# vt-asaplab/porla

Measured on NVIDIA B200. Metric: G1 MSM points/sec, higher is better.
Workload: dtype u32 (8x32-bit limb Montgomery, IMAD carry chains)

## Files before the change

porla_b200/csrc/msm_impl.cuh:

```cuda
#pragma once
#include <atomic>
#include <cstdio>
#include <cstdlib>
#include <mutex>
#include <type_traits>

#include "arena.h"
#include "msm.h"
#include "msm_kernels.cuh"
#include "small_kernels.cuh"
#include "affine_kernels.cuh"

namespace porla {

extern std::atomic<uint64_t> g_launches;
#define LAUNCHED() (g_launches.fetch_add(1, std::memory_order_relaxed))



template <class C> struct CurveIdOf;
template <> struct CurveIdOf<Bn254> { static constexpr int value = kCurveBn254; };
template <> struct CurveIdOf<Secp256k1> { static constexpr int value = kCurveSecp256k1; };

template <class C>
void import_into_impl(const uint8_t* d_bytes, int fmt, uint32_t n, void* d_points_out, uint8_t* d_flags_out,
                      cudaStream_t stream, bool with_phi) {
    using F = typename C::F;
    if (!n) return;
    int mask = C::F::Params::kMontgomery ? 1 : 0;
    k_import_points<C><<<(n + 127) / 128, 128, 0, stream>>>(d_bytes, fmt, mask, n, reinterpret_cast<Affine<F>*>(d_points_out),
                                                           d_flags_out, nullptr);
    LAUNCHED();
    if constexpr (C::kGlv) {
        if (with_phi) {
            k_phi_table<C><<<(n + 127) / 128, 128, 0, stream>>>(reinterpret_cast<const Affine<F>*>(d_points_out), n,
                                                               reinterpret_cast<F*>(reinterpret_cast<Affine<F>*>(d_points_out) + n));
            LAUNCHED();
        }
    }
    PORLA_CUDA(cudaGetLastError());
}

template <class C>
void import_impl(const uint8_t* d_bytes, int fmt, uint32_t n, PointTable* out, cudaStream_t stream) {
    using F = typename C::F;
    Affine<F>* pts = nullptr;
    uint8_t* flags = nullptr;
    uint32_t* d_count = nullptr;
    PORLA_CUDA(cudaMalloc(&pts, (size_t)(n ? n : 1) * (sizeof(Affine<F>) + (C::kGlv ? sizeof(F) : 0))));
    PORLA_CUDA(cudaMalloc(&flags, (size_t)(n ? n : 1)));
    PORLA_CUDA(cudaMalloc(&d_count, 4));
    PORLA_CUDA(cudaMemsetAsync(d_count, 0, 4, stream));
    if (n) {
        int mask = C::F::Params::kMontgomery ? 1 : 0;
        k_import_points<C><<<(n + 127) / 128, 128, 0, stream>>>(d_bytes, fmt, mask, n, pts, flags, d_count);
        LAUNCHED();
        if constexpr (C::kGlv) {
            k_phi_table<C><<<(n + 127) / 128, 128, 0, stream>>>(pts, n, reinterpret_cast<F*>(pts + n));
            LAUNCHED();
        }
        PORLA_CUDA(cudaGetLastError());
    }
    uint32_t h_count = 0;
    PORLA_CUDA(cudaMemcpyAsync(&h_count, d_count, 4, cudaMemcpyDeviceToHost, stream));
    PORLA_CUDA(cudaStreamSynchronize(stream));
    PORLA_CUDA(cudaFree(d_count));
    out->d_points = pts;
    out->n = n;
    out->n_inf = h_count;
    out->curve = CurveIdOf<C>::value;
    out->phi_off = C::kGlv ? n : 0u;
    out->d_phi_x = C::kGlv ? static_cast<void*>(pts + n) : nullptr;
    if (h_count == 0) {
        PORLA_CUDA(cudaFree(flags));
        out->d_flags = nullptr;
    } else {
        out->d_flags = flags;
    }
}

template <class C>
void msm_small_impl(const PointTable& table, const uint8_t* d_scalars, uint32_t n, uint32_t nbatch, const MsmOptions& opt,
                    const MsmPlan& plan, uint8_t* d_out, void* d_out_xyzz, cudaStream_t stream) {
    using F = typename C::F;
    using XC = XYZZ<typename C::FC>;
    const bool lut = plan.mode == kPlanLut;
    const uint32_t slots = nbatch * (uint32_t)plan.nwin;
    uint32_t K = 1, nblk;
    if (lut) {
        uint32_t per_thread = 1;
        if (nbatch > 8) {
            const uint64_t want_threads = 148ull * 3 * kTreeThreads * 4;
            per_thread = (uint32_t)(((uint64_t)n * nbatch) / want_threads);
            if (per_thread < 1) per_thread = 1;
            if (per_thread > 16) per_thread = 16;
            while (per_thread > 1 && n / per_thread < (uint32_t)kTreeThreads) per_thread >>= 1;
        }
        K = nbatch > 8 ? (uint32_t)table.fb_nwin * per_thread : 2u;
        const uint32_t threads = (n * (uint32_t)table.fb_nwin + K - 1) / K;
        nblk = (threads + kTreeThreads - 1) / kTreeThreads;
    } else {
        nblk = (n + 2 * kTreeThreads - 1) / (2 * kTreeThreads);
    }
    if (!nblk) nblk = 1;
    const size_t need = Arena::padded((size_t)slots * nblk, sizeof(XYZZ<F>)) + Arena::padded(slots, 4) +
                        Arena::padded(slots, sizeof(XYZZ<F>)) + 1024;
    DeviceCtx& cx = device_ctx();
    Arena& g_arena = cx.arena;
    StageTimer& g_stage_timer = cx.timer;
    std::unique_lock<std::mutex> lock(cx.engine_mu, std::defer_lock);
    XYZZ<F>* partials;
    uint32_t* tickets;
    XYZZ<F>* wsum;
    if (opt.d_scratch && need <= opt.scratch_bytes) {
        uint8_t* b = reinterpret_cast<uint8_t*>(opt.d_scratch);
        partials = reinterpret_cast<XYZZ<F>*>(b);
        b += Arena::padded((size_t)slots * nblk, sizeof(XYZZ<F>));
        tickets = reinterpret_cast<uint32_t*>(b);
        b += Arena::padded(slots, 4);
        wsum = reinterpret_cast<XYZZ<F>*>(b);
    } else {
        lock.lock();
        g_arena.acquire(stream);
        g_arena.reserve(need, stream);
        g_arena.reset();
        partials = g_arena.take<XYZZ<F>>((size_t)slots * nblk);
        tickets = g_arena.take<uint32_t>(slots);
        wsum = g_arena.take<XYZZ<F>>(slots);
    }
    for (int st = kStageCount; st <= kStageAccumulate; st++) g_stage_timer.mark(st, stream);
    if (nblk > 1) PORLA_CUDA(cudaMemsetAsync(tickets, 0, (size_t)slots * 4, stream));
    if (lut) {
        const int m_major = nbatch > 8 ? 1 : 0;
        k_lut_sum<C><<<m_major ? dim3(nbatch, nblk) : dim3(nblk, nbatch), kTreeThreads, 0, stream>>>(
            reinterpret_cast<const Affine<F>*>(table.d_lut), table.fb_c, table.fb_nwin, d_scalars, opt.scalar_be, n, K, m_major,
            partials, tickets, wsum);
    } else {
        k_small_bits<C><<<dim3(nblk, (uint32_t)plan.nwin, nbatch), kTreeThreads, 0, stream>>>(
            reinterpret_cast<const Affine<F>*>(table.d_points), table.d_flags, d_scalars, opt.scalar_be, n, opt.shared_points,
            partials, tickets, wsum);
    }
    LAUNCHED();
    g_stage_timer.mark(kStageReduce, stream);
    g_stage_timer.mark(kStageFinalize, stream);
    if (opt.d_window_sums) {
        PORLA_CUDA(cudaMemcpyAsync(opt.d_window_sums, wsum, (size_t)slots * sizeof(XYZZ<F>), cudaMemcpyDeviceToDevice, stream));
    } else {
        k_finalize<C><<<(nbatch + 31) / 32, 32, 0, stream>>>((const XC*)wsum, nbatch, plan.nwin, plan.c, opt.out_fmt, d_out,
                                                            reinterpret_cast<XC*>(d_out_xyzz));
        LAUNCHED();
    }
    g_stage_timer.mark(kNumStages, stream);
    if (lock.owns_lock()) g_arena.release(stream);
    PORLA_CUDA(cudaGetLastError());
}

template <class C>
void msm_impl(const PointTable& table, const uint8_t* d_scalars, uint32_t n, uint32_t nbatch,
                     const MsmOptions& opt, uint8_t* d_out, void* d_out_xyzz, cudaStream_t stream) {
    using F = typename C::F;
    const int curve = CurveIdOf<C>::value;
    {
        const MsmPlan plan = msm_plan_table(table, n, nbatch, opt);
        if (plan.mode != kPlanPipeline && n > 0) {
            msm_small_impl<C>(table, d_scalars, n, nbatch, opt, plan, d_out, d_out_xyzz, stream);
            return;
        }
    }
    MsmShape sh;
    sh.n = n;
    sh.nbatch = nbatch;
    sh.shared = opt.shared_points ? 1u : 0u;
    const bool streamed = opt.part_mode != kPartWhole;
    if (streamed && (nbatch != 1 || !opt.d_buckets || opt.window_bits <= 0 || opt.glv < 0 || !opt.no_fixed_base)) {
        fprintf(stderr, "[libmultiexp/porla_b200] FATAL: a streamed MSM part needs one MSM, a shared bucket array and a forced window layout\n");
        abort();
    }
    const bool fixed = table.fb_c > 0 && opt.shared_points && !opt.no_fixed_base &&
                       (opt.window_bits == 0 || opt.window_bits == table.fb_c);
    const MsmPlan wplan = fixed ? MsmPlan{table.fb_c, 1, kPlanPipeline, 0} : msm_plan(curve, n, nbatch, opt.window_bits, opt.glv);
    const bool glv = wplan.glv != 0;
    if (glv && !(C::kGlv && table.phi_off && table.d_phi_x)) {
        fprintf(stderr, "[libmultiexp/porla_b200] FATAL: GLV plan for a table without its endomorphism image\n");
        abort();
    }
    sh.c = wplan.c;
    sh.nwin = glv ? 2 * wplan.nwin : (C::kScalarBits + 1 + sh.c - 1) / sh.c;
    int slice_shift = 0;
    while ((1 << slice_shift) < opt.slice_count) slice_shift++;
    if (opt.slice_count > 1) {
        const bool ok = (1 << slice_shift) == opt.slice_count && opt.slice_index >= 0 && opt.slice_index < opt.slice_count &&
                        !fixed && nbatch == 1 && opt.window_bits > 0 && opt.glv >= 0 && opt.no_fixed_base &&
                        msm_max_slices(wplan, opt.slice_count) == opt.slice_count;
        if (!ok) {
            fprintf(stderr, "[libmultiexp/porla_b200] FATAL: bucket slice %d of %d: needs one MSM, a forced window layout and a power-of-two "
                            "slice count that leaves whole coarse bins (c = %d)\n", opt.slice_index, opt.slice_count, wplan.c);
            abort();
        }
    }
    sh.slice_shift = (uint32_t)slice_shift;
    sh.slice_r = opt.slice_count > 1 ? (uint32_t)opt.slice_index : 0u;
    sh.nbuckets = (1u << (sh.c - 1)) >> slice_shift;
    sh.fixed_n = fixed ? table.fb_n : 0u;
    sh.glv_wh = glv ? wplan.nwin : 0;
    sh.phi_off = glv ? table.phi_off : 0u;
    const int slot_windows = fixed ? 1 : (glv ? wplan.nwin : sh.nwin);

    const uint64_t slots = (uint64_t)nbatch * slot_windows;
    const uint64_t nbt64 = slots * sh.nbuckets;
    const uint64_t pairs64 = (uint64_t)nbatch * n * sh.nwin;
    if (nbt64 >= (1ull << 32) || pairs64 >= (1ull << 32) || (uint64_t)nbatch * n >= (1ull << 31) ||
        (fixed && (uint64_t)table.fb_n * sh.nwin >= (1ull << 31))) {
        fprintf(stderr, "[libmultiexp/porla_b200] FATAL: MSM shape too large for 32-bit indexing\n");
        abort();
    }
    const uint32_t nbt = (uint32_t)nbt64;
    const uint32_t ntiles = (nbt + kScanTile - 1) / kScanTile;

    uint32_t chunk = 64;
    while (chunk > 4 && (uint64_t)nbt / chunk < 24576ull) chunk >>= 1;
    while (chunk > 4 && sh.nbuckets / chunk < 4) chunk >>= 1;
    if (const char* e = getenv("PORLA_REDUCE_CHUNK")) { if (atoi(e) >= 1) chunk = (uint32_t)atoi(e); }
    if (chunk > sh.nbuckets) chunk = sh.nbuckets;
    uint32_t threads_per_slot = (sh.nbuckets + chunk - 1) / chunk;
    uint32_t blocks_per_slot = (threads_per_slot + kRedThreads - 1) / kRedThreads;
    static const uint64_t quad_max = [] { const char* e = getenv("PORLA_REDUCE_QUAD_MAX"); return e ? (uint64_t)atoll(e) : (uint64_t)C::kReduceQuadMax; }();
    static const uint64_t quad_target = [] { const char* e = getenv("PORLA_REDUCE_QUADS"); return e && atoll(e) > 0 ? (uint64_t)atoll(e) : 148ull * kQuadsPerBlock; }();
    const bool reduce_v1 = getenv("PORLA_REDUCE_V1") != nullptr || (uint64_t)nbt > quad_max;
    uint32_t log_m = 0;
    while (log_m < 6 && ((uint64_t)nbt >> log_m) > quad_target) log_m++;
    while ((sh.nbuckets >> log_m) > (uint32_t)(kTopMaxBlocks * kQuadsPerBlock)) log_m++;
    while (log_m > 0 && (1u << log_m) > sh.nbuckets) log_m--;
    const uint32_t scan_tps = sh.nbuckets >> log_m;
    const uint32_t scan_group = scan_tps >= (uint32_t)kQuadsPerBlock ? (uint32_t)kQuadsPerBlock : scan_tps;
    const uint32_t scan_bps = scan_tps >= (uint32_t)kQuadsPerBlock ? scan_tps / kQuadsPerBlock : 1u;
    if (!reduce_v1) blocks_per_slot = 2 * scan_bps;

    const uint64_t pairs_cap = pairs64 ? pairs64 : 1;
    const uint64_t pairs_geo = (pairs_cap >> slice_shift) ? (pairs_cap >> slice_shift) : 1;
    const uint64_t wave = 148ull * 4ull * kAccThreads;
    const uint64_t waves = (pairs_geo + wave * 64 - 1) / (wave * 64);
    uint32_t L = (uint32_t)((pairs_geo + waves * wave - 1) / (waves * wave));
    if (waves == 1) {
        const uint64_t l2 = pairs_geo / (wave * 18 / 25);
        if (l2 >= 16 && l2 <= 64) L = (uint32_t)l2;
    }
    if (L < 16) L = 16;
    if (L > 64) L = 64;
    if (const char* e = getenv("PORLA_SLICE_LEN")) { if (atoi(e) >= 2) L = (uint32_t)atoi(e); }
    int aff_rounds = 0;
    {
        const char* e = getenv("PORLA_ACC_AFFINE");
        const bool big = pairs_cap >= (uint64_t)148 * PORLA_AFF_MIN_BLOCKS * kAffThreads * kAffL * 2;
        const int want = e ? atoi(e) : (big ? kAffDefaultRounds : 0);
        if (want > 0 && !streamed && slice_shift == 0) {
            aff_rounds = want > 2 ? 2 : want;
            L = kAffL;
        }
    }
    const uint32_t nslices_cap = (uint32_t)((pairs_cap + L - 1) / L);
    const uint32_t serial_limit = (nslices_cap >> slice_shift) < 200000u ? kStitchSerialSmall : kStitchSerial;
    const uint32_t long_cap = (uint32_t)(pairs_cap / ((uint64_t)L * serial_limit)) + 2;

    const bool radix = nbatch == 1 && n >= (1u << 19) && sh.nwin <= 28 && sh.c >= 9 && sh.c <= 20 && (sh.nbuckets >> (sh.c / 2)) <= (uint32_t)kPartMaxBins && !getenv("PORLA_ATOMIC_SCATTER");
    const int lb = sh.c / 2;
    const uint32_t ncoarse = radix ? (nbt >> lb) : 0u;
    DeviceCtx& cx = device_ctx();
    Arena& g_arena = cx.arena;
    StageTimer& g_stage_timer = cx.timer;
    std::lock_guard<std::mutex> lock(cx.engine_mu);
    size_t need = (radix ? Arena::padded(pairs_cap, 8) + Arena::padded(ncoarse, 4) : 0) + Arena::padded(nbt, 4) * 2 + Arena::padded(ntiles + 1, 4) + 512 +
                  Arena::padded(pairs_cap, 8) + (streamed ? 0 : Arena::padded(nbt, sizeof(XYZZ<F>))) +
                  2 * Arena::padded(nslices_cap, sizeof(XYZZ<F>)) + Arena::padded(long_cap, 8) +
                  Arena::padded(slots * blocks_per_slot, sizeof(XYZZ<F>)) + Arena::padded(slots, sizeof(XYZZ<F>));
    g_arena.acquire(stream);
    g_arena.reserve(need, stream);
    g_arena.reset();
    uint32_t* counters = g_arena.take<uint32_t>(nbt);
    uint32_t* offsets = g_arena.take<uint32_t>(nbt);
    uint32_t* tile_sums = g_arena.take<uint32_t>(ntiles + 1);
    uint32_t* grand = g_arena.take<uint32_t>(1);
    uint32_t* long_count = g_arena.take<uint32_t>(1);
    uint2* sorted = g_arena.take<uint2>(pairs_cap);
    uint2* part = radix ? g_arena.take<uint2>(pairs_cap) : nullptr;
    uint32_t* coarse_cursor = radix ? g_arena.take<uint32_t>(ncoarse) : nullptr;
    XYZZ<F>* buckets = streamed ? reinterpret_cast<XYZZ<F>*>(opt.d_buckets) : g_arena.take<XYZZ<F>>(nbt);
    const int into = opt.part_mode == kPartMiddle || opt.part_mode == kPartLast;
    XYZZ<F>* part_head = g_arena.take<XYZZ<F>>(nslices_cap);
    XYZZ<F>* part_tail = g_arena.take<XYZZ<F>>(nslices_cap);
    uint2* long_runs = g_arena.take<uint2>(long_cap);
    XYZZ<F>* partials = g_arena.take<XYZZ<F>>(slots * blocks_per_slot);
    XYZZ<F>* wsum = g_arena.take<XYZZ<F>>(slots);

    const Affine<F>* points = reinterpret_cast<const Affine<F>*>(fixed ? table.d_fb_points : table.d_points);
    using FC = typename C::FC;
    using XC = XYZZ<FC>;
    static_assert(sizeof(XC) == sizeof(XYZZ<F>), "layouts must coincide");
    const uint64_t total_scalars = (uint64_t)n * nbatch;

    g_stage_timer.mark(kStageCount, stream);
    const char* sv2 = getenv("PORLA_SORT_V2");
    const bool v2_fits = ncoarse > 0 && pairs_cap / ncoarse <= (uint64_t)(kBigBin * 0.95);
    const bool sort_v2 = radix && slice_shift == 0 && lb <= 10 && (size_t)ncoarse * 4 <= (160u << 10) && (sv2 ? sv2[0] == '1' : v2_fits);
    PORLA_CUDA(cudaMemsetAsync(counters, 0, (size_t)nbt * 4, stream));
    PORLA_CUDA(cudaMemsetAsync(grand, 0, 4, stream));
    PORLA_CUDA(cudaMemsetAsync(long_count, 0, 4, stream));
    static_assert(sizeof(XYZZ<F>) == 128, "k_fine_smem / k_big_scan clear 128-byte bucket records");
    if (!into && !sort_v2) PORLA_CUDA(cudaMemsetAsync(buckets, 0, (size_t)nbt * sizeof(XYZZ<F>), stream));
    uint4* zero_buckets = into ? nullptr : reinterpret_cast<uint4*>(buckets);
    if (total_scalars && sort_v2) {
        static std::once_flag attr_once_dev2[kMaxDevices];
        const size_t smem0 = (size_t)ncoarse * 4;
        const size_t smem1 = ((size_t)9 * kPartTile + 2 * kPartMaxBins) * 4 + (size_t)kPartTile * 8;
        const size_t smem2 = (size_t)2 * kFineHist * 4 + (size_t)kFineTile * 8;
        const size_t smem3 = (size_t)kBigBin * 6 + (size_t)kFineLocalBuckets * 4;
        std::call_once(attr_once_dev2[current_device()], [=] {
            PORLA_CUDA(cudaFuncSetAttribute(k_coarse_count<C, false>, cudaFuncAttributeMaxDynamicSharedMemorySize, 160 << 10));
            PORLA_CUDA(cudaFuncSetAttribute(k_partition_coarse<C, false>, cudaFuncAttributeMaxDynamicSharedMemorySize, (int)smem1));
            if constexpr (C::kGlv) {
                PORLA_CUDA(cudaFuncSetAttribute(k_coarse_count<C, true>, cudaFuncAttributeMaxDynamicSharedMemorySize, 160 << 10));
                PORLA_CUDA(cudaFuncSetAttribute(k_partition_coarse<C, true>, cudaFuncAttributeMaxDynamicSharedMemorySize, (int)smem1));
            }
            PORLA_CUDA(cudaFuncSetAttribute(k_partition_fine_big, cudaFuncAttributeMaxDynamicSharedMemorySize, (int)smem2));
            PORLA_CUDA(cudaFuncSetAttribute(k_fine_smem, cudaFuncAttributeMaxDynamicSharedMemorySize, (int)smem3));
        });
        uint32_t* coarse_count = offsets;
        uint32_t* coarse_off = offsets + ncoarse + 1;
        PORLA_CUDA(cudaMemsetAsync(coarse_count, 0, (size_t)(ncoarse + 1) * 4, stream));
        uint32_t cgrid = (uint32_t)((total_scalars + kCoarseCountThreads - 1) / kCoarseCountThreads);
        if (cgrid > 148u * 2u) cgrid = 148u * 2u;
        bool glv_done = false;
        if constexpr (C::kGlv) {
            if (glv) {
                k_coarse_count<C, true><<<cgrid, kCoarseCountThreads, smem0, stream>>>(d_scalars, opt.scalar_be, table.d_flags, sh, lb, ncoarse, coarse_count);
                glv_done = true;
            }
        }
        if (!glv_done)
            k_coarse_count<C, false><<<cgrid, kCoarseCountThreads, smem0, stream>>>(d_scalars, opt.scalar_be, table.d_flags, sh, lb, ncoarse, coarse_count);
        LAUNCHED();
        g_stage_timer.mark(kStageScan, stream);
        k_coarse_scan<<<1, 1024, 0, stream>>>(coarse_count, ncoarse, coarse_off, coarse_cursor, grand);
        LAUNCHED();
        g_stage_timer.mark(kStageScatter, stream);
        glv_done = false;
        if constexpr (C::kGlv) {
            if (glv) {
                k_partition_coarse<C, true><<<(n + kPartTile - 1) / kPartTile, kPartThreads, smem1, stream>>>(
                    d_scalars, opt.scalar_be, table.d_flags, sh, lb, coarse_cursor, part);
                glv_done = true;
            }
        }
        if (!glv_done)
            k_partition_coarse<C, false><<<(n + kPartTile - 1) / kPartTile, kPartThreads, smem1, stream>>>(
                d_scalars, opt.scalar_be, table.d_flags, sh, lb, coarse_cursor, part);
        LAUNCHED();
        k_fine_smem<<<ncoarse, kFineSmemThreads, smem3, stream>>>(part, coarse_off, lb, sorted, zero_buckets);
        LAUNCHED();
        const uint32_t tiles = (uint32_t)((pairs_cap + kFineTile - 1) / kFineTile);
        k_big_count<<<tiles, kFineThreads, 0, stream>>>(part, grand, coarse_off, lb, counters);
        LAUNCHED();
        k_big_scan<<<ncoarse, kFineLocalThreads, 0, stream>>>(coarse_off, lb, counters, zero_buckets);
        LAUNCHED();
        k_partition_fine_big<<<tiles, kFineThreads, smem2, stream>>>(part, grand, coarse_off, lb, counters, sorted);
        LAUNCHED();
    } else if (total_scalars) {
        uint32_t grid = (uint32_t)((total_scalars + 255) / 256);
        if (grid > 148u * 32u) grid = 148u * 32u;
        bool launched_glv = false;
        if constexpr (C::kGlv) {
            if (glv) {
                k_digits<C, false, true><<<grid, 256, 0, stream>>>(d_scalars, opt.scalar_be, table.d_flags, sh, 0, sh.nwin, counters, nullptr);
                launched_glv = true;
            }
        }
        if (!launched_glv)
            k_digits<C, false, false><<<grid, 256, 0, stream>>>(d_scalars, opt.scalar_be, table.d_flags, sh, 0, sh.nwin, counters, nullptr);
        LAUNCHED();
        g_stage_timer.mark(kStageScan, stream);
        k_scan_tiles<<<ntiles, kScanThreads, 0, stream>>>(counters, offsets, nbt, tile_sums);
        LAUNCHED();
        k_scan_sums<<<1, kScanThreads, 0, stream>>>(tile_sums, ntiles, grand);
        LAUNCHED();
        k_scan_add<<<ntiles, kScanThreads, 0, stream>>>(offsets, counters, nbt, tile_sums);
        LAUNCHED();
        g_stage_timer.mark(kStageScatter, stream);
        if (radix) {
            static std::once_flag attr_once_dev[kMaxDevices];
            std::once_flag& attr_once = attr_once_dev[current_device()];
            const size_t smem1 = ((size_t)9 * kPartTile + 2 * kPartMaxBins) * 4 + (size_t)kPartTile * 8;
            const size_t smem2 = (size_t)2 * kFineHist * 4 + (size_t)kFineTile * 8;
            std::call_once(attr_once, [=] {
                PORLA_CUDA(cudaFuncSetAttribute(k_partition_coarse<C, false>, cudaFuncAttributeMaxDynamicSharedMemorySize, (int)smem1));
                if constexpr (C::kGlv)
                    PORLA_CUDA(cudaFuncSetAttribute(k_partition_coarse<C, true>, cudaFuncAttributeMaxDynamicSharedMemorySize, (int)smem1));
                PORLA_CUDA(cudaFuncSetAttribute(k_partition_fine, cudaFuncAttributeMaxDynamicSharedMemorySize, (int)smem2));
            });
            k_init_coarse<<<(ncoarse + 255) / 256, 256, 0, stream>>>(offsets, nbt, lb, ncoarse, coarse_cursor);
            LAUNCHED();
            bool coarse_glv = false;
            if constexpr (C::kGlv) {
                if (glv) {
                    k_partition_coarse<C, true><<<(n + kPartTile - 1) / kPartTile, kPartThreads, smem1, stream>>>(
                        d_scalars, opt.scalar_be, table.d_flags, sh, lb, coarse_cursor, part);
                    coarse_glv = true;
                }
            }
            if (!coarse_glv)
                k_partition_coarse<C, false><<<(n + kPartTile - 1) / kPartTile, kPartThreads, smem1, stream>>>(
                    d_scalars, opt.scalar_be, table.d_flags, sh, lb, coarse_cursor, part);
            LAUNCHED();
            k_partition_fine<<<(uint32_t)((pairs_cap + kFineTile - 1) / kFineTile), kFineThreads, smem2, stream>>>(part, grand, lb,
                                                                                                             counters, sorted);
            LAUNCHED();
        } else {
        int wgroup = sh.nwin;
        if (nbatch == 1) {
            uint64_t per_window = (uint64_t)n * 8;
            wgroup = (int)((64ull << 20) / (per_window ? per_window : 1));
            if (wgroup < 1) wgroup = 1;
            if (wgroup > sh.nwin) wgroup = sh.nwin;
        }
        for (int w0 = 0; w0 < sh.nwin; w0 += wgroup) {
            int w1 = w0 + wgroup < sh.nwin ? w0 + wgroup : sh.nwin;
            bool scatter_glv = false;
            if constexpr (C::kGlv) {
                if (glv) {
                    k_digits<C, true, true><<<grid, 256, 0, stream>>>(d_scalars, opt.scalar_be, table.d_flags, sh, w0, w1, counters, sorted);
                    scatter_glv = true;
                }
            }
            if (!scatter_glv)
                k_digits<C, true, false><<<grid, 256, 0, stream>>>(d_scalars, opt.scalar_be, table.d_flags, sh, w0, w1, counters, sorted);
            LAUNCHED();
        }
        }
    }
    if (total_scalars) {
        g_stage_timer.mark(kStageAccumulate, stream);
        if (aff_rounds > 0)
            k_accumulate_affine<C><<<(nslices_cap + kAffThreads - 1) / kAffThreads, kAffThreads, 0, stream>>>(
                points, reinterpret_cast<const F*>(table.d_phi_x), sh.phi_off, sorted, grand, buckets, part_head, part_tail, aff_rounds);
        else
            k_accumulate<C><<<(nslices_cap + kAccThreads - 1) / kAccThreads, kAccThreads, 0, stream>>>(
                points, reinterpret_cast<const F*>(table.d_phi_x), sh.phi_off, sorted, grand, L, buckets, part_head, part_tail, into);
        LAUNCHED();
        if (getenv("PORLA_STITCH_COMPACT"))
            k_stitch<C, FC><<<(nslices_cap + 63) / 64, 64, 0, stream>>>(sorted, grand, L, (XC*)buckets, (const XC*)part_head,
                                                                       (const XC*)part_tail, long_count, long_runs, serial_limit);
        else
            k_stitch<C, F><<<(nslices_cap + 63) / 64, 64, 0, stream>>>(sorted, grand, L, buckets, part_head, part_tail,
                                                                      long_count, long_runs, serial_limit);
        LAUNCHED();
        k_stitch_long<C><<<148, kLongThreads, 0, stream>>>(sorted, grand, L, (XC*)buckets, (const XC*)part_head, long_count,
                                                          long_runs);
        LAUNCHED();
    } else {
        g_stage_timer.mark(kStageScan, stream);
        g_stage_timer.mark(kStageScatter, stream);
        g_stage_timer.mark(kStageAccumulate, stream);
    }
    g_stage_timer.mark(kStageReduce, stream);
    if (opt.part_mode == kPartFirst || opt.part_mode == kPartMiddle) {
        g_stage_timer.mark(kStageFinalize, stream);
        g_stage_timer.mark(kNumStages, stream);
        g_arena.release(stream);
        PORLA_CUDA(cudaGetLastError());
        return;
    }
    if (slots * blocks_per_slot >= (1ull << 31)) {
        fprintf(stderr, "[libmultiexp/porla_b200] FATAL: too many window slots for one launch\n");
        abort();
    }
    const XYZZ<F>* window_sums = partials;
    if (reduce_v1) {
        const uint32_t rgrid = threads_per_slot >= (uint32_t)kRedThreads
                                   ? (uint32_t)(slots * blocks_per_slot)
                                   : (uint32_t)((slots + kRedThreads / threads_per_slot - 1) / (kRedThreads / threads_per_slot));
        k_reduce<C><<<rgrid, kRedThreads, 0, stream>>>((const XC*)buckets, sh.nbuckets, chunk, threads_per_slot, (uint32_t)slots,
                                                       (XC*)partials, sh.slice_shift, sh.slice_r);
        LAUNCHED();
        if (blocks_per_slot > 1) {
            k_window_sums<C><<<(uint32_t)slots, kRedThreads, 0, stream>>>((const XC*)partials, blocks_per_slot, (XC*)wsum);
            LAUNCHED();
            window_sums = wsum;
        }
    } else {
        XYZZ<F>* out_w = partials;
        XYZZ<F>* out_s = out_w + slots * scan_bps;
        const uint32_t sgrid = scan_group == (uint32_t)kQuadsPerBlock
                                   ? (uint32_t)(slots * scan_bps)
                                   : (uint32_t)((slots + kQuadsPerBlock / scan_group - 1) / (kQuadsPerBlock / scan_group));
        k_reduce_scan<C><<<sgrid, kQuadThreads, 0, stream>>>(buckets, sh.nbuckets, log_m, scan_group, (uint32_t)slots, out_w, out_s);
        LAUNCHED();
        if (scan_bps > 1 || sh.slice_shift != 0) {
            uint32_t log_u = log_m;
            while ((1u << log_u) < ((uint32_t)kQuadsPerBlock << log_m)) log_u++;
            k_reduce_top<C><<<(uint32_t)slots, kQuadThreads, 0, stream>>>(out_w, out_s, scan_bps, log_u, sh.slice_shift, sh.slice_r, wsum);
            LAUNCHED();
            window_sums = wsum;
        }
    }
    g_stage_timer.mark(kStageFinalize, stream);
    if (opt.d_window_sums) {
        PORLA_CUDA(cudaMemcpyAsync(opt.d_window_sums, window_sums, slots * sizeof(XYZZ<F>), cudaMemcpyDeviceToDevice, stream));
    } else {
        k_finalize<C><<<(nbatch + 31) / 32, 32, 0, stream>>>((const XC*)window_sums, nbatch, slot_windows, sh.c, opt.out_fmt, d_out,
                                                            reinterpret_cast<XC*>(d_out_xyzz));
        LAUNCHED();
    }
    g_stage_timer.mark(kNumStages, stream);
    g_arena.release(stream);
    PORLA_CUDA(cudaGetLastError());
}

template <class C>
void precompute_impl(PointTable* t, int c, cudaStream_t stream) {
    using FC = typename C::FC;
    const int nwin = (C::kScalarBits + 1 + c - 1) / c;
    if (t->d_fb_points) PORLA_CUDA(cudaFree(t->d_fb_points));
    void* out = nullptr;
    PORLA_CUDA(cudaMalloc(&out, (size_t)nwin * (t->n ? t->n : 1) * sizeof(Affine<FC>)));
    if (t->n) {
        k_precompute_windows<C><<<(t->n + 127) / 128, 128, 0, stream>>>(reinterpret_cast<const Affine<FC>*>(t->d_points), t->n, c, nwin,
                                                                      reinterpret_cast<Affine<FC>*>(out));
        LAUNCHED();
        PORLA_CUDA(cudaGetLastError());
    }
    t->d_fb_points = out;
    t->fb_c = c;
    t->fb_nwin = nwin;
    t->fb_n = t->n;
    if (t->d_lut) PORLA_CUDA(cudaFree(t->d_lut));
    t->d_lut = nullptr;
}

template <class C>
void lut_impl(PointTable* t, cudaStream_t stream) {
    using FC = typename C::FC;
    if (!t->n || !t->d_fb_points) return;
    void* out = nullptr;
    const size_t entries = ((size_t)t->fb_nwin * t->n) << (t->fb_c - 1);
    PORLA_CUDA(cudaMalloc(&out, entries * sizeof(Affine<FC>)));
    const uint32_t threads = t->n * (uint32_t)t->fb_nwin;
    k_lut_build<C><<<(threads + 127) / 128, 128, 0, stream>>>(reinterpret_cast<const Affine<FC>*>(t->d_fb_points), t->d_flags, t->n,
                                                             t->fb_c, t->fb_nwin, reinterpret_cast<Affine<FC>*>(out));
    LAUNCHED();
    PORLA_CUDA(cudaGetLastError());
    t->d_lut = out;
}

template <class C>
void combine_impl(const void* d_parts, uint32_t count, uint32_t nbatch, int out_fmt, uint8_t* d_out, cudaStream_t stream) {
    using F = typename C::FC;
    k_combine<C><<<(nbatch + 63) / 64, 64, 0, stream>>>(reinterpret_cast<const XYZZ<F>*>(d_parts), count, nbatch, out_fmt, d_out);
    LAUNCHED();
    PORLA_CUDA(cudaGetLastError());
}

template <class C>
void scalar_mul_impl(const PointTable& table, const uint8_t* d_scalars, int scalar_be, uint32_t n, void* d_out_affine,
                     cudaStream_t stream) {
    using F = typename C::FC;
    k_scalar_mul<C><<<(n + 127) / 128, 128, 0, stream>>>(reinterpret_cast<const Affine<F>*>(table.d_points), table.n, d_scalars,
                                                        scalar_be, n, reinterpret_cast<Affine<F>*>(d_out_affine));
    LAUNCHED();
    PORLA_CUDA(cudaGetLastError());
}

template <class C>
void butterfly_impl(PointTable* t, uint32_t m, const uint8_t* d_twiddles, int scalar_be, cudaStream_t stream) {
    const uint32_t nb = t->n / 2;
    if (!nb) return;
    if (!t->d_flags) {
        PORLA_CUDA(cudaMalloc(&t->d_flags, t->n));
        PORLA_CUDA(cudaMemsetAsync(t->d_flags, 0, t->n, stream));
    }
    const char* force = getenv("PORLA_BUTTERFLY_FIELD");
    const bool inlined = force ? force[0] == 'i' : (C::kGlv || nb < 148u * 512u);
    const char* fg = getenv("PORLA_BUTTERFLY_GLV");
    const bool glv = C::kGlv && (fg ? fg[0] == '1' : true);
    auto* pf = reinterpret_cast<Affine<typename C::F>*>(t->d_points);
    auto* pc = reinterpret_cast<Affine<typename C::FC>*>(t->d_points);
    const dim3 grid((nb + 127) / 128);
    const char* fq = getenv("PORLA_BUTTERFLY_QUAD");
    bool quad = false;
    if constexpr (C::kGlv) quad = glv && (fq ? fq[0] == '1' : nb <= 9472u);
    if (quad) {
        if constexpr (C::kGlv) k_butterfly_quad<C><<<(nb * 4 + kBflyQuadThreads - 1) / kBflyQuadThreads, kBflyQuadThreads, 0, stream>>>(pf, t->d_flags, t->n, m, d_twiddles, scalar_be);
    } else if (inlined && glv) k_butterfly<C, typename C::F, true><<<grid, 128, 0, stream>>>(pf, t->d_flags, t->n, m, d_twiddles, scalar_be);
    else if (inlined) k_butterfly<C, typename C::F, false><<<grid, 128, 0, stream>>>(pf, t->d_flags, t->n, m, d_twiddles, scalar_be);
    else if (glv) k_butterfly<C, typename C::FC, true><<<grid, 128, 0, stream>>>(pc, t->d_flags, t->n, m, d_twiddles, scalar_be);
    else k_butterfly<C, typename C::FC, false><<<grid, 128, 0, stream>>>(pc, t->d_flags, t->n, m, d_twiddles, scalar_be);
    LAUNCHED();
    if constexpr (C::kGlv) {
        if (t->phi_off) {
            k_phi_table<C><<<(t->n + 127) / 128, 128, 0, stream>>>(reinterpret_cast<const Affine<typename C::F>*>(t->d_points), t->n,
                                                                  reinterpret_cast<typename C::F*>(t->d_phi_x));
            LAUNCHED();
        }
    }
    PORLA_CUDA(cudaGetLastError());
}

template <class C>
// ... 60 lines not shown
```

porla_b200/csrc/msm_kernels.cuh:

```cuda
#pragma once
#include "ec.cuh"
#include "quad.cuh"

namespace porla {

enum ScalarFormat : int { kScalarBE32 = 0, kScalarLE32 = 1 };
enum PointFormat : int { kPointBE64 = 0, kPointLE64 = 1 };

struct MsmShape {
    uint32_t n;
    uint32_t nbatch;
    uint32_t shared;
    int c;
    int nwin;
    uint32_t nbuckets;
    uint32_t fixed_n;
    int glv_wh;
    uint32_t phi_off;
    uint32_t slice_shift;
    uint32_t slice_r;
};

PORLA_D uint32_t slice_bucket(const MsmShape& sh, uint32_t mag) {
    const uint32_t b = mag - 1u;
// ... 832 lines not shown
        }
        const uint32_t ex = block_exclusive_scan(v, &total);
        if (i < nb) c[i] = carry + ex;
        carry += total;
        __syncthreads();
    }
}

static __global__ void __launch_bounds__(kFineThreads, 3)
k_partition_fine_big(const uint2* __restrict__ part, const uint32_t* __restrict__ total_pairs, const uint32_t* __restrict__ coarse_off,
                     int lb, uint32_t* __restrict__ cursor, uint2* __restrict__ sorted) {
    extern __shared__ uint32_t smem[];
    uint32_t* cnt = smem;
    uint32_t* delta = cnt + kFineHist;
    uint2* stage = reinterpret_cast<uint2*>(delta + kFineHist);
    __shared__ uint32_t s_total;
    const uint32_t M = *total_pairs;
    const uint64_t lo64 = (uint64_t)blockIdx.x * kFineTile;
    if (lo64 >= M) return;
    const uint32_t lo = (uint32_t)lo64;
    const uint32_t hi = M - lo > (uint32_t)kFineTile ? lo + kFineTile : M;
    const uint32_t bin_lo = __ldg(&part[lo].x) >> lb, bin_hi = __ldg(&part[hi - 1].x) >> lb;
    bool any = false;
    for (uint32_t b = bin_lo; b <= bin_hi && !any; b++) any = bin_is_big(coarse_off, b);
    if (!any) return;
    for (uint32_t b = threadIdx.x; b < kFineHist; b += kFineThreads) cnt[b] = 0;
    const uint32_t kbase = bin_lo << lb;
    __syncthreads();
    uint2 e[kFinePerThread];
    uint32_t rank[kFinePerThread];
#pragma unroll
    for (int q = 0; q < kFinePerThread; q++) {
        const uint32_t idx = lo + q * kFineThreads + threadIdx.x;
        e[q] = make_uint2(0xffffffffu, 0u);
        if (idx < hi) {
            const uint2 v = __ldg(&part[idx]);
            if (bin_is_big(coarse_off, v.x >> lb)) {
                e[q] = v;
                const uint32_t rel = v.x - kbase;
                if (rel < kFineHist) rank[q] = atomicAdd(&cnt[rel], 1u);
            }
        }
    }
    __syncthreads();
    {
        constexpr uint32_t ept = kFineHist / kFineThreads;
        uint32_t v[ept], sum = 0;
        const uint32_t b0 = threadIdx.x * ept;
#pragma unroll
        for (uint32_t k = 0; k < ept; k++) {
            v[k] = cnt[b0 + k];
            sum += v[k];
        }
        uint32_t ex = block_exclusive_scan(sum, &s_total);
#pragma unroll
        for (uint32_t k = 0; k < ept; k++) {
            cnt[b0 + k] = ex;
            delta[b0 + k] = v[k] ? atomicAdd(&cursor[kbase + b0 + k], v[k]) - ex : 0u;
            ex += v[k];
        }
    }
    __syncthreads();
#pragma unroll
    for (int q = 0; q < kFinePerThread; q++) {
        if (e[q].x == 0xffffffffu) continue;
        const uint32_t rel = e[q].x - kbase;
        if (rel < kFineHist) stage[cnt[rel] + rank[q]] = e[q];
        else sorted[atomicAdd(&cursor[e[q].x], 1u)] = e[q];
    }
    __syncthreads();
    const uint32_t total = s_total;
    for (uint32_t j = threadIdx.x; j < total; j += kFineThreads) {
        const uint2 x = stage[j];
        sorted[delta[x.x - kbase] + j] = x;
    }
}

constexpr int kAccThreads = 128;
#ifndef PORLA_ACC_MIN_BLOCKS
#define PORLA_ACC_MIN_BLOCKS 4
#endif

template <class C>
PORLA_D Affine<typename C::F> load_signed_point(const Affine<typename C::F>* __restrict__ points,
                                                const typename C::F* __restrict__ phi_x, uint32_t phi_off, uint32_t e) {
    using F = typename C::F;
    const uint32_t idx = e & 0x7fffffffu;
    const bool image = C::kGlv && phi_off != 0 && idx >= phi_off;
    const uint32_t j = image ? idx - phi_off : idx;
    const uint4* sx = image ? reinterpret_cast<const uint4*>(phi_x + j) : reinterpret_cast<const uint4*>(points + j);
    const uint4* sy = reinterpret_cast<const uint4*>(points + j) + 2;
    Affine<F> p;
    uint4* d = reinterpret_cast<uint4*>(&p);
    d[0] = __ldg(sx);
    d[1] = __ldg(sx + 1);
    d[2] = __ldg(sy);
    d[3] = __ldg(sy + 1);
    if (e >> 31) p.y = p.y.neg();
    return p;
}

template <class F>
PORLA_D XYZZ<F> bucket_seed(const XYZZ<F>* __restrict__ buckets, uint32_t key, int into) {
    XYZZ<F> acc = XYZZ<F>::inf();
    if (into) {
        const uint4* s = reinterpret_cast<const uint4*>(buckets + key);
        uint4* d = reinterpret_cast<uint4*>(&acc);
#pragma unroll
        for (int i = 0; i < 8; i++) d[i] = s[i];
    }
    return acc;
}

template <class C>
__global__ void __launch_bounds__(kAccThreads, PORLA_ACC_MIN_BLOCKS)
k_accumulate(const Affine<typename C::F>* __restrict__ points, const typename C::F* __restrict__ phi_x, uint32_t phi_off,
             const uint2* __restrict__ sorted, const uint32_t* __restrict__ total_pairs, uint32_t L,
             XYZZ<typename C::F>* __restrict__ buckets, XYZZ<typename C::F>* __restrict__ part_head,
             XYZZ<typename C::F>* __restrict__ part_tail, int into) {
    using F = typename C::F;
    const uint32_t M = *total_pairs;
    const uint32_t t = blockIdx.x * blockDim.x + threadIdx.x;
    const uint64_t start64 = (uint64_t)t * L;
    if (start64 >= M) return;
    const uint32_t start = (uint32_t)start64;
    const uint32_t end = (M - start > L) ? start + L : M;
    const uint32_t prev_key = start > 0 ? __ldg(&sorted[start - 1].x) : 0xffffffffu;
    const uint32_t next_key = end < M ? __ldg(&sorted[end].x) : 0xffffffffu;

    uint32_t key = __ldg(&sorted[start].x);
    bool first = true;
    XYZZ<F> acc = prev_key == key ? XYZZ<F>::inf() : bucket_seed<F>(buckets, key, into);
    for (uint32_t pos = start; pos < end; ++pos) {
        const uint2 e = __ldg(&sorted[pos]);
        const Affine<F> q = load_signed_point<C>(points, phi_x, phi_off, e.y);
        if (e.x != key) {
            if (first && prev_key == key) st16(part_head + t, acc);
            else st16(buckets + key, acc);
            first = false;
            key = e.x;
            acc = bucket_seed<F>(buckets, key, into);
        }
        if (acc.is_inf()) acc = XYZZ<F>{q.x, q.y, F::one(), F::one()};
        else acc.madd_finite(q);
    }
    if (first && prev_key == key) st16(part_head + t, acc);
    else if (next_key == key) st16(part_tail + t, acc);
    else st16(buckets + key, acc);
}

constexpr uint32_t kStitchSerial = 48;
constexpr uint32_t kStitchSerialSmall = 8;

template <class C, class F>
__global__ void __launch_bounds__(64)
k_stitch(const uint2* __restrict__ sorted, const uint32_t* __restrict__ total_pairs, uint32_t L,
         XYZZ<F>* __restrict__ buckets, const XYZZ<F>* __restrict__ part_head,
         const XYZZ<F>* __restrict__ part_tail, uint32_t* __restrict__ long_count,
         uint2* __restrict__ long_runs, uint32_t serial_limit) {
    const uint32_t M = *total_pairs;
    const uint32_t t = blockIdx.x * blockDim.x + threadIdx.x;
    const uint64_t start64 = (uint64_t)t * L;
    if (start64 >= M) return;
    const uint32_t start = (uint32_t)start64;
    if (M - start <= L) return;
    const uint32_t end = start + L;
    const uint32_t key = __ldg(&sorted[end - 1].x);
    if (__ldg(&sorted[end].x) != key) return;
    if (__ldg(&sorted[start].x) == key && start > 0 && __ldg(&sorted[start - 1].x) == key) return;
    const uint32_t nslices = (uint32_t)(((uint64_t)M + L - 1) / L);
    uint32_t u = t + 1, cnt = 0;
    XYZZ<F> acc = ld16(part_tail + t);
    for (;;) {
        if (cnt == serial_limit) {
            st16(buckets + key, acc);
            uint32_t slot = atomicAdd(long_count, 1u);
            long_runs[slot] = make_uint2(key, u);
            return;
        }
        acc.add(ld16(part_head + u));
        cnt++;
        uint32_t uend = (u + 1 < nslices) ? (u + 1) * L : M;
        if (u + 1 < nslices && __ldg(&sorted[uend - 1].x) == key && __ldg(&sorted[uend].x) == key) u++;
        else break;
    }
    st16(buckets + key, acc);
}

constexpr int kLongThreads = 128;

template <class C>
__global__ void __launch_bounds__(kLongThreads)
k_stitch_long(const uint2* __restrict__ sorted, const uint32_t* __restrict__ total_pairs, uint32_t L,
              XYZZ<typename C::FC>* __restrict__ buckets, const XYZZ<typename C::FC>* __restrict__ part_head,
              const uint32_t* __restrict__ long_count, const uint2* __restrict__ long_runs) {
    using F = typename C::FC;
    __shared__ XYZZ<F> sh[kLongThreads];
    __shared__ uint32_t s_last;
    const uint32_t M = *total_pairs;
    const uint32_t nruns = *long_count;
    const uint32_t nslices = (uint32_t)(((uint64_t)M + L - 1) / L);
    for (uint32_t r = blockIdx.x; r < nruns; r += gridDim.x) {
        const uint32_t key = long_runs[r].x, u0 = long_runs[r].y;
        if (threadIdx.x == 0) {
            uint32_t lo = u0 * L, hi = M;
            while (hi - lo > 1) {
                uint32_t mid = lo + (hi - lo) / 2;
                if (__ldg(&sorted[mid].x) == key) lo = mid;
                else hi = mid;
            }
            s_last = lo / L;
        }
        __syncthreads();
        const uint32_t last = s_last < nslices ? s_last : nslices - 1;
        XYZZ<F> acc = XYZZ<F>::inf();
        for (uint32_t u = u0 + threadIdx.x; u <= last; u += kLongThreads) acc.add(ld16(part_head + u));
        sh[threadIdx.x] = acc;
        __syncthreads();
        for (int o = kLongThreads / 2; o > 0; o >>= 1) {
            if ((int)threadIdx.x < o) {
                XYZZ<F> a = sh[threadIdx.x];
                a.add(sh[threadIdx.x + o]);
                sh[threadIdx.x] = a;
            }
            __syncthreads();
        }
        if (threadIdx.x == 0) {
            XYZZ<F> a = ld16(buckets + key);
            a.add(sh[0]);
            st16(buckets + key, a);
        }
        __syncthreads();
    }
}

constexpr int kRedThreads = 64;

template <class C>
__global__ void __launch_bounds__(kRedThreads)
k_reduce(const XYZZ<typename C::FC>* __restrict__ buckets, uint32_t nb, uint32_t chunk,
         uint32_t threads_per_slot, uint32_t total_slots, XYZZ<typename C::FC>* __restrict__ partials,
         uint32_t slice_shift, uint32_t slice_r) {
    using F = typename C::FC;
    __shared__ XYZZ<F> sh[kRedThreads];
    uint32_t slot, t, group;
    size_t out_index;
    if (threads_per_slot >= kRedThreads) {
        const uint32_t blocks_per_slot = (threads_per_slot + kRedThreads - 1) / kRedThreads;
        slot = blockIdx.x / blocks_per_slot;
        const uint32_t blk = blockIdx.x - slot * blocks_per_slot;
        t = blk * kRedThreads + threadIdx.x;
        group = kRedThreads;
        out_index = (size_t)slot * blocks_per_slot + blk;
    } else {
        const uint32_t slots_per_block = kRedThreads / threads_per_slot;
        slot = blockIdx.x * slots_per_block + threadIdx.x / threads_per_slot;
        t = threadIdx.x % threads_per_slot;
        group = threads_per_slot;
        out_index = slot;
    }
    XYZZ<F> acc = XYZZ<F>::inf();
    if (slot < total_slots && t < threads_per_slot) {
        const XYZZ<F>* base = buckets + (size_t)slot * nb;
        uint32_t lo = t * chunk;
        uint32_t hi = lo + chunk < nb ? lo + chunk : nb;
        XYZZ<F> run = XYZZ<F>::inf();
        for (uint32_t k = hi; k-- > lo;) {
            XYZZ<F> bk = ld16(base + k);
            run.add(bk);
            acc.add(run);
        }
        if (slice_shift == 0) {
            if (lo != 0) {
                XYZZ<F> w = mul_small(run, lo);
                acc.add(w);
            }
        } else {
            acc.add(run.neg());
            for (uint32_t d = 0; d < slice_shift; d++) acc = acc.dbl();
            XYZZ<F> w = mul_small(run, (lo << slice_shift) + slice_r + 1u);
            acc.add(w);
        }
    }
    sh[threadIdx.x] = acc;
    __syncthreads();
    const uint32_t local = threadIdx.x % group;
    for (uint32_t o = group / 2; o > 0; o >>= 1) {
        if (local < o) {
            XYZZ<F> a = sh[threadIdx.x];
            a.add(sh[threadIdx.x + o]);
            sh[threadIdx.x] = a;
        }
        __syncthreads();
    }
    if (local == 0 && slot < total_slots) st16(partials + out_index, sh[threadIdx.x]);
}

constexpr int kQuadsPerBlock = 64;
constexpr int kQuadThreads = 4 * kQuadsPerBlock;
constexpr int kTopMaxBlocks = kQuadsPerBlock * 64;

template <class F>
__device__ __noinline__ QuadPoint<F> quad_add_nl(QuadPoint<F> a, QuadPoint<F> b) { return quad_add(a, b); }
template <class F>
__device__ __noinline__ QuadPoint<F> quad_dbl_nl(QuadPoint<F> a) { return quad_dbl(a); }

template <class F>
PORLA_D QuadPoint<F> quad_from_shared(const XYZZ<F>* p) { return QuadPoint<F>{reinterpret_cast<const F*>(p)[threadIdx.x & 3]}; }
template <class F>
PORLA_D void quad_to_shared(XYZZ<F>* p, const QuadPoint<F>& v) { reinterpret_cast<F*>(p)[threadIdx.x & 3] = v.c; }

template <class F>
PORLA_D void quad_tree_sum(XYZZ<F>* sh, uint32_t q, uint32_t l, uint32_t count) {
    for (uint32_t o = count / 2; o > 0; o >>= 1) {
        const bool act = l < o;
        if (__any_sync(kFullMask, act)) {
            QuadPoint<F> x = QuadPoint<F>::inf(), y = QuadPoint<F>::inf();
            if (act) {
                x = quad_from_shared(&sh[q]);
                y = quad_from_shared(&sh[q + o]);
            }
            x = quad_add_nl(x, y);
            if (act) quad_to_shared(&sh[q], x);
        }
        __syncthreads();
    }
}

template <class F>
PORLA_D QuadPoint<F> quad_suffix_scan(XYZZ<F>* sh, uint32_t q, uint32_t l, uint32_t count, QuadPoint<F> a) {
    quad_to_shared(&sh[q], a);
    __syncthreads();
    for (uint32_t d = 1; d < count; d <<= 1) {
        const bool has = l + d < count;
        QuadPoint<F> b = QuadPoint<F>::inf();
        if (has) b = quad_from_shared(&sh[q + d]);
        __syncthreads();
        a = quad_add_nl(a, b);
        if (has) quad_to_shared(&sh[q], a);
        __syncthreads();
    }
    return a;
}

template <class C>
__global__ void __launch_bounds__(kQuadThreads)
k_reduce_scan(XYZZ<typename C::F>* buckets, uint32_t nb, uint32_t log_m, uint32_t group, uint32_t total_slots,
              XYZZ<typename C::F>* __restrict__ out_w, XYZZ<typename C::F>* __restrict__ out_s) {
    using F = typename C::F;
    using Q = QuadPoint<F>;
    __shared__ XYZZ<F> sh[kQuadsPerBlock];
    const uint32_t m = 1u << log_m;
    const uint32_t q = threadIdx.x >> 2;
    uint32_t slot, blk, blocks_per_slot;
    if (group == (uint32_t)kQuadsPerBlock) {
        blocks_per_slot = (nb >> log_m) / kQuadsPerBlock;
        slot = blockIdx.x / blocks_per_slot;
        blk = blockIdx.x - slot * blocks_per_slot;
    } else {
        blocks_per_slot = 1;
        slot = blockIdx.x * (kQuadsPerBlock / group) + q / group;
        blk = 0;
    }
    const uint32_t l = q & (group - 1);
    const bool live = slot < total_slots;
    XYZZ<F>* base = buckets + (size_t)slot * nb + (size_t)blk * ((size_t)group << log_m);
    XYZZ<F>* p = base + ((size_t)l << log_m);
    Q a = Q::inf(), nxt = Q::inf();
    if (live) {
        a = Q::load_coherent(p + (m - 1));
        if (m > 1) nxt = Q::load_coherent(p + (m - 2));
    }
    for (uint32_t k = m - 1; k-- > 0;) {
        const Q b = nxt;
        if (live && k > 0) nxt = Q::load_coherent(p + (k - 1));
        a = quad_add_nl(a, b);
        if (live) a.store(p + k);
    }
    a = quad_suffix_scan(sh, q, l, group, a);
    if (l == 0 && live) a.store(out_s + (size_t)slot * blocks_per_slot + blk);
    Q v = l != 0 ? a : Q::inf();
    for (uint32_t d = 0; d < log_m; d++) v = quad_dbl_nl(v);
    nxt = Q::inf();
    if (live) nxt = Q::load_coherent(base + l);
    for (uint32_t i = 0; i < m; i++) {
        const Q b = nxt;
        if (live && i + 1 < m) nxt = Q::load_coherent(base + l + (size_t)(i + 1) * group);
        v = quad_add_nl(v, b);
    }
    __syncthreads();
    quad_to_shared(&sh[q], v);
    __syncthreads();
    quad_tree_sum(sh, q, l, group);
    if (l == 0 && live) quad_from_shared(&sh[q]).store(out_w + (size_t)slot * blocks_per_slot + blk);
}

template <class C>
__global__ void __launch_bounds__(kQuadThreads)
k_reduce_top(const XYZZ<typename C::F>* __restrict__ in_w, const XYZZ<typename C::F>* __restrict__ in_s, uint32_t nblk_in,
             uint32_t log_u, uint32_t slice_shift, uint32_t slice_r, XYZZ<typename C::F>* __restrict__ wsum) {
    using F = typename C::F;
    using Q = QuadPoint<F>;
    __shared__ XYZZ<F> sh[kQuadsPerBlock];
    const uint32_t b = threadIdx.x >> 2;
    const uint32_t per = nblk_in > (uint32_t)kQuadsPerBlock ? nblk_in / kQuadsPerBlock : 1u;
    const uint32_t nblk = nblk_in / per;
    const bool live = b < nblk;
    const size_t at = (size_t)blockIdx.x * nblk_in + (size_t)b * per;
    Q a = Q::inf();
    Q wq = Q::inf();
    if (per == 1) {
        if (live) {
            a = Q::load(in_s + at);
            wq = Q::load(in_w + at);
        }
    } else {
        Q z = Q::inf();
        for (uint32_t j = per; j-- > 0;) {
            Q s = Q::inf(), w = Q::inf();
            if (live) {
                s = Q::load(in_s + at + j);
                w = Q::load(in_w + at + j);
            }
            a = quad_add_nl(a, s);
            wq = quad_add_nl(wq, w);
            if (j != 0) z = quad_add_nl(z, a);
        }
        for (uint32_t d = 0; d < log_u; d++) z = quad_dbl_nl(z);
        wq = quad_add_nl(wq, z);
        for (uint32_t q = per; q > 1; q >>= 1) log_u++;
    }
    a = quad_suffix_scan(sh, b, b, nblk, a);
    const Q g = quad_from_shared(&sh[0]);
    Q v = (b != 0 && live) ? a : Q::inf();
    for (uint32_t d = 0; d < log_u; d++) v = quad_dbl_nl(v);
    v = quad_add_nl(v, wq);
    __syncthreads();
    quad_to_shared(&sh[b], v);
    __syncthreads();
    quad_tree_sum(sh, b, b, nblk);
    if (threadIdx.x < 32) {
        Q z = quad_from_shared(&sh[0]);
        if (slice_shift != 0) {
            for (uint32_t d = 0; d < slice_shift; d++) z = quad_dbl_nl(z);
            const uint32_t k = (1u << slice_shift) - 1u - slice_r;
            Q t = Q::inf();
            for (int bit = 3; bit >= 0; bit--) {
                t = quad_dbl_nl(t);
                t = quad_add_nl(t, ((k >> bit) & 1u) ? g : Q::inf());
            }
            if ((threadIdx.x & 3) == 1) t.c = t.c.neg();
            z = quad_add_nl(z, t);
        }
        if (b == 0) z.store(wsum + blockIdx.x);
    }
}

template <class C>
__global__ void __launch_bounds__(kRedThreads)
k_window_sums(const XYZZ<typename C::FC>* __restrict__ partials, uint32_t count,
              XYZZ<typename C::FC>* __restrict__ wsum) {
    using F = typename C::FC;
    __shared__ XYZZ<F> sh[kRedThreads];
    const XYZZ<F>* p = partials + (size_t)blockIdx.x * count;
    XYZZ<F> acc = XYZZ<F>::inf();
    for (uint32_t k = threadIdx.x; k < count; k += kRedThreads) acc.add(ld16(p + k));
    sh[threadIdx.x] = acc;
    __syncthreads();
    for (int o = kRedThreads / 2; o > 0; o >>= 1) {
        if ((int)threadIdx.x < o) {
            XYZZ<F> a = sh[threadIdx.x];
            a.add(sh[threadIdx.x + o]);
            sh[threadIdx.x] = a;
        }
        __syncthreads();
    }
    if (threadIdx.x == 0) st16(wsum + blockIdx.x, sh[0]);
}

template <class C>
__global__ void __launch_bounds__(32)
k_finalize(const XYZZ<typename C::FC>* __restrict__ wsums, uint32_t nbatch, int nwin, int c, int out_fmt,
           uint8_t* __restrict__ out, XYZZ<typename C::FC>* __restrict__ out_xyzz) {
    using F = typename C::FC;
    const uint32_t m = blockIdx.x * blockDim.x + threadIdx.x;
    if (m >= nbatch) return;
    const XYZZ<F>* ws = wsums + (size_t)m * nwin;
    XYZZ<F> r = XYZZ<F>::inf();
    for (int w = nwin - 1; w >= 0; w--) {
        if (!r.is_inf())
            for (int k = 0; k < c; k++) r = r.dbl();
        r.add(ld16(ws + w));
    }
    if (out_xyzz) st16(out_xyzz + m, r);
    if (out) {
        Affine<F> a = r.to_affine();
        F x = a.x.from_internal(), y = a.y.from_internal();
// ... 496 lines not shown
```

Before: 309.9 million.

## Lengthen accumulate slices and add quad-thread stitch kernel for small slice counts

Slice length for the accumulate kernel may now reach 224 instead of 64, with the wave count capped at a minimum of eight. This cuts the number of slices and the partial-sum stitching work. A new k_stitch_quad kernel spreads each stitch chain's point additions across four cooperating threads and is used when there are at most 65536 slices. The compact-format stitch path is removed. Longer slices trade more serial work per thread and possible load imbalance for fewer partials.

```diff
diff --git a/porla_b200/csrc/msm_impl.cuh b/porla_b200/csrc/msm_impl.cuh
--- a/porla_b200/csrc/msm_impl.cuh
+++ b/porla_b200/csrc/msm_impl.cuh
@@ -17,6 +17,9 @@
 #define LAUNCHED() (g_launches.fetch_add(1, std::memory_order_relaxed))
 
 
+
+constexpr uint64_t kMinAccWaves = 8;
+constexpr uint32_t kMaxSliceLen = 224;
 
 template <class C> struct CurveIdOf;
 template <> struct CurveIdOf<Bn254> { static constexpr int value = kCurveBn254; };
@@ -239,14 +242,16 @@
     const uint64_t pairs_cap = pairs64 ? pairs64 : 1;
     const uint64_t pairs_geo = (pairs_cap >> slice_shift) ? (pairs_cap >> slice_shift) : 1;
     const uint64_t wave = 148ull * 4ull * kAccThreads;
-    const uint64_t waves = (pairs_geo + wave * 64 - 1) / (wave * 64);
+    uint64_t waves = (pairs_geo + wave * kMaxSliceLen - 1) / (wave * kMaxSliceLen);
+    const uint64_t waves64 = (pairs_geo + wave * 64 - 1) / (wave * 64);
+    if (waves < kMinAccWaves) waves = waves64 < kMinAccWaves ? waves64 : kMinAccWaves;
     uint32_t L = (uint32_t)((pairs_geo + waves * wave - 1) / (waves * wave));
     if (waves == 1) {
         const uint64_t l2 = pairs_geo / (wave * 18 / 25);
         if (l2 >= 16 && l2 <= 64) L = (uint32_t)l2;
     }
     if (L < 16) L = 16;
-    if (L > 64) L = 64;
+    if (L > kMaxSliceLen) L = kMaxSliceLen;
     if (const char* e = getenv("PORLA_SLICE_LEN")) { if (atoi(e) >= 2) L = (uint32_t)atoi(e); }
     int aff_rounds = 0;
     {
@@ -445,12 +450,12 @@
             k_accumulate<C><<<(nslices_cap + kAccThreads - 1) / kAccThreads, kAccThreads, 0, stream>>>(
                 points, reinterpret_cast<const F*>(table.d_phi_x), sh.phi_off, sorted, grand, L, buckets, part_head, part_tail, into);
         LAUNCHED();
-        if (getenv("PORLA_STITCH_COMPACT"))
-            k_stitch<C, FC><<<(nslices_cap + 63) / 64, 64, 0, stream>>>(sorted, grand, L, (XC*)buckets, (const XC*)part_head,
-                                                                       (const XC*)part_tail, long_count, long_runs, serial_limit);
+        if (nslices_cap <= kStitchQuadMaxSlices)
+            k_stitch_quad<C><<<(nslices_cap + kStitchQuads - 1) / kStitchQuads, 4 * kStitchQuads, 0, stream>>>(
+                sorted, grand, L, buckets, part_head, part_tail, long_count, long_runs, serial_limit);
         else
-            k_stitch<C, F><<<(nslices_cap + 63) / 64, 64, 0, stream>>>(sorted, grand, L, buckets, part_head, part_tail,
-                                                                      long_count, long_runs, serial_limit);
+            k_stitch<C><<<(nslices_cap + 63) / 64, 64, 0, stream>>>(sorted, grand, L, buckets, part_head, part_tail,
+                                                                   long_count, long_runs, serial_limit);
         LAUNCHED();
         k_stitch_long<C><<<148, kLongThreads, 0, stream>>>(sorted, grand, L, (XC*)buckets, (const XC*)part_head, long_count,
                                                           long_runs);
diff --git a/porla_b200/csrc/msm_kernels.cuh b/porla_b200/csrc/msm_kernels.cuh
--- a/porla_b200/csrc/msm_kernels.cuh
+++ b/porla_b200/csrc/msm_kernels.cuh
@@ -1008,12 +1008,13 @@
 constexpr uint32_t kStitchSerial = 48;
 constexpr uint32_t kStitchSerialSmall = 8;
 
-template <class C, class F>
+template <class C>
 __global__ void __launch_bounds__(64)
 k_stitch(const uint2* __restrict__ sorted, const uint32_t* __restrict__ total_pairs, uint32_t L,
-         XYZZ<F>* __restrict__ buckets, const XYZZ<F>* __restrict__ part_head,
-         const XYZZ<F>* __restrict__ part_tail, uint32_t* __restrict__ long_count,
+         XYZZ<typename C::F>* __restrict__ buckets, const XYZZ<typename C::F>* __restrict__ part_head,
+         const XYZZ<typename C::F>* __restrict__ part_tail, uint32_t* __restrict__ long_count,
          uint2* __restrict__ long_runs, uint32_t serial_limit) {
+    using F = typename C::F;
     const uint32_t M = *total_pairs;
     const uint32_t t = blockIdx.x * blockDim.x + threadIdx.x;
     const uint64_t start64 = (uint64_t)t * L;
@@ -1199,6 +1200,52 @@
     return a;
 }
 
+constexpr uint32_t kStitchQuadMaxSlices = 65536;
+constexpr int kStitchQuads = 16;
+
+template <class C>
+__global__ void __launch_bounds__(4 * kStitchQuads, 8)
+k_stitch_quad(const uint2* __restrict__ sorted, const uint32_t* __restrict__ total_pairs, uint32_t L,
+         XYZZ<typename C::F>* __restrict__ buckets, const XYZZ<typename C::F>* __restrict__ part_head,
+         const XYZZ<typename C::F>* __restrict__ part_tail, uint32_t* __restrict__ long_count,
+         uint2* __restrict__ long_runs, uint32_t serial_limit) {
+    using Q = QuadPoint<typename C::F>;
+    const uint32_t M = *total_pairs;
+    const uint32_t t = blockIdx.x * kStitchQuads + (threadIdx.x >> 2);
+    const uint64_t start64 = (uint64_t)t * L;
+    bool own = start64 < M && M - (uint32_t)start64 > L;
+    uint32_t key = 0;
+    if (own) {
+        const uint32_t start = (uint32_t)start64, end = start + L;
+        key = __ldg(&sorted[end - 1].x);
+        own = __ldg(&sorted[end].x) == key &&
+              !(__ldg(&sorted[start].x) == key && start > 0 && __ldg(&sorted[start - 1].x) == key);
+    }
+    if (!__any_sync(kFullMask, own)) return;
+    const uint32_t nslices = (uint32_t)(((uint64_t)M + L - 1) / L);
+    uint32_t u = t + 1, cnt = 0;
+    bool more = own, handed = false;
+    Q acc = own ? Q::load(part_tail + t) : Q::inf();
+    while (__any_sync(kFullMask, more)) {
+        if (more && cnt == serial_limit) {
+            more = false;
+            handed = true;
+        }
+        const Q b = more ? Q::load(part_head + u) : Q::inf();
+        acc = quad_add_nl(acc, b);
+        if (more) {
+            cnt++;
+            const uint32_t uend = (u + 1 < nslices) ? (u + 1) * L : M;
+            if (u + 1 < nslices && __ldg(&sorted[uend - 1].x) == key && __ldg(&sorted[uend].x) == key) u++;
+            else more = false;
+        }
+    }
+    if (own) {
+        acc.store(buckets + key);
+        if (handed && (threadIdx.x & 3) == 0) long_runs[atomicAdd(long_count, 1u)] = make_uint2(key, u);
+    }
+}
+
 template <class C>
 __global__ void __launch_bounds__(kQuadThreads)
 k_reduce_scan(XYZZ<typename C::F>* buckets, uint32_t nb, uint32_t log_m, uint32_t group, uint32_t total_slots,
```

Result: no change. 309.6 million (median of 6 runs) (-0.1%).
